# adamgreig/basebandboard

Hardware: AMD Instinct MI355X
Metric: awgn_clt_gsamples_per_s (higher is better)
Workload: dtype u32 bit-sliced GF(2) / int8 out

## Files before the change

basebandboard_amd/_lib.py:

```python
import ctypes as C
import pathlib

import torch

_HERE = pathlib.Path(__file__).resolve().parent
LIB_PATH = _HERE / "libbbb_hip.so"

SHARD_TRIALS, SHARD_SEEDS, SHARD_BITS, SHARD_GROUPS = 0, 1, 2, 3
BBB_OK, BBB_EINVAL, BBB_ENOMEM, BBB_EHIP, BBB_EIO, BBB_ENODEV, BBB_EUNSUP = 0, -1, -2, -3, -4, -5, -6

SYMBOLS = [
    "bbb_abi_version", "bbb_strerror", "bbb_last_error_detail", "bbb_device_count", "bbb_free",
    "bbb_lutopt_load_matrix_file", "bbb_lutopt_create", "bbb_lutopt_destroy", "bbb_lutopt_set_stream",
    "bbb_lutopt_is_specialised", "bbb_lutopt_set_staged", "bbb_lutopt_set_custom_fill", "bbb_lutopt_set_custom_ber", "bbb_lutopt_attach_custom_library", "bbb_lutopt_profile", "bbb_lutopt_profile_read", "bbb_lutopt_profile_read_mover", "bbb_lutopt_state_at", "bbb_lutopt_fill_words", "bbb_awgn_fill_i8", "bbb_awgn_fill_i16", "bbb_awgn_prefetch", "bbb_awgn_stream_open", "bbb_awgn_stream_next", "bbb_awgn_stream_read", "bbb_awgn_stream_seek", "bbb_awgn_stream_tell", "bbb_awgn_stream_close", "bbb_awgn_hist",
    "bbb_clt_tree_i16", "bbb_prbs_fill", "bbb_prbs_fill_hint", "bbb_prbs_check", "bbb_prbs_check_dev", "bbb_prbs_state_at",
    "bbb_prbs_detector_run", "bbb_prbs_detector_stream", "bbb_ber_trials", "bbb_ber_trials_dev", "bbb_ber_run_open", "bbb_ber_run_next", "bbb_ber_run_next_dev", "bbb_ber_run_tell", "bbb_ber_run_close", "bbb_ber_sweep_multi", "bbb_sweep_shard", "bbb_multi_last_info", "bbb_multi_release", "bbb_shaper_fill_i16", "bbb_tx_fill_i16", "bbb_tx_stream_open", "bbb_tx_stream_next", "bbb_tx_stream_read", "bbb_tx_stream_seek", "bbb_tx_stream_tell", "bbb_tx_stream_close", "bbb_rx_slice", "bbb_rx_phase_search", "bbb_eye_accumulate_i16", "bbb_tx_eye_open", "bbb_tx_eye_run", "bbb_tx_eye_close", "bbb_tx_ber_sweep_open", "bbb_tx_ber_sweep_run", "bbb_tx_ber_sweep_close", "bbb_acf_accumulate_i16", "bbb_tx_acf_open", "bbb_tx_acf_run", "bbb_tx_acf_close", "bbb_nco_rom", "bbb_nco_open", "bbb_nco_set_cfg", "bbb_nco_set_stream", "bbb_nco_run", "bbb_nco_get_state", "bbb_nco_set_state", "bbb_nco_close", "bbb_sinc_coefficients", "bbb_sinc_interpolate", "bbb_sinc_eye_open", "bbb_sinc_eye_run", "bbb_sinc_eye_close", "bbb_fir_moving_average", "bbb_fir_filter", "bbb_fir_slice", "bbb_link_sweep_open", "bbb_link_sweep_run", "bbb_link_sweep_close", "bbb_gf2_berlekamp_massey", "bbb_gf2_recur",
    "bbb_gf2_dot", "bbb_gf2_poly_is_primitive", "bbb_gf2_poly_modexp", "bbb_lutopt_charpoly", "bbb_lutopt_is_full_period",
    "bbb_lutopt_save_matrix_file", "bbb_lutopt_search_candidate", "bbb_lutopt_search",
    "bbb_errstat_open", "bbb_errstat_accumulate", "bbb_errstat_skip", "bbb_errstat_read", "bbb_errstat_reset",
    "bbb_errstat_set_stream", "bbb_errstat_geometry", "bbb_errstat_close",
    "bbb_xcorr_accumulate_i16", "bbb_tx_xcorr_open", "bbb_tx_xcorr_run", "bbb_tx_xcorr_close",
    "bbb_ddc_run", "bbb_ddc_polar_host",
    "bbb_dfe_run", "bbb_dfe_geometry", "bbb_dfe_model_host",
]


class BbbError(RuntimeError):
    def __init__(self, code, what, detail):
        super().__init__(f"{what}: {detail}" if detail else what)
        self.code = code


class TrialCfg(C.Structure):
    _fields_ = [("prbs_k", C.c_int32), ("amp", C.c_int32), ("noise_var", C.c_int32), ("reserved", C.c_int32),
                ("prbs_state", C.c_uint64), ("warmup", C.c_uint64), ("first_bit", C.c_uint64),
                ("nbits", C.c_uint64)]

# ... 98 lines not shown
            f"{LIB_PATH} is missing: build it with `python -c 'import __graft_entry__ as g; g.build()'` "
            "(hipcc --offload-arch=gfx950).  basebandboard_amd has no CPU fallback.")
    l = C.CDLL(str(LIB_PATH))
    vp, u64, i32 = C.c_void_p, C.c_uint64, C.c_int
    u64p = C.POINTER(C.c_uint64)
    l.bbb_abi_version.restype = i32
    l.bbb_strerror.restype = C.c_char_p
    l.bbb_strerror.argtypes = [i32]
    l.bbb_last_error_detail.restype = C.c_char_p
    l.bbb_device_count.argtypes = [C.POINTER(i32)]
    l.bbb_free.argtypes = [vp]
    l.bbb_free.restype = None
    l.bbb_lutopt_load_matrix_file.argtypes = [C.c_char_p, C.POINTER(i32), C.POINTER(C.POINTER(C.c_uint16)),
                                              C.POINTER(C.POINTER(C.c_uint32))]
    l.bbb_lutopt_create.argtypes = [C.POINTER(vp), i32, C.POINTER(C.c_uint16), C.POINTER(C.c_uint32), u64p, i32]
    l.bbb_lutopt_destroy.argtypes = [vp]
    l.bbb_lutopt_set_stream.argtypes = [vp, vp]
    l.bbb_lutopt_is_specialised.argtypes = [vp]
    l.bbb_lutopt_set_staged.argtypes = [vp, i32]
    l.bbb_lutopt_state_at.argtypes = [vp, u64, u64p]
    l.bbb_lutopt_profile.argtypes = [vp, i32]
    l.bbb_lutopt_profile_read.argtypes = [vp, C.POINTER(C.c_double), C.POINTER(C.c_double), u64p, i32]
    l.bbb_lutopt_profile_read_mover.argtypes = [vp, C.POINTER(C.c_double), u64p, i32]
    l.bbb_lutopt_fill_words.argtypes = [vp, vp, u64, u64, i32]
    l.bbb_awgn_fill_i8.argtypes = [vp, vp, u64, u64]
    l.bbb_awgn_fill_i16.argtypes = [vp, vp, u64, u64]
    l.bbb_awgn_prefetch.argtypes = [vp, u64, u64]
    l.bbb_awgn_stream_open.argtypes = [vp, u64, u64, i32, C.POINTER(vp)]
    l.bbb_awgn_stream_next.argtypes = [vp, vp]
    l.bbb_awgn_stream_read.argtypes = [vp, vp, u64]
    l.bbb_awgn_stream_seek.argtypes = [vp, u64]
    l.bbb_awgn_stream_tell.argtypes = [vp, u64p]
    l.bbb_awgn_stream_close.argtypes = [vp]
    l.bbb_awgn_hist.argtypes = [vp, vp, u64, u64]
    l.bbb_clt_tree_i16.argtypes = [i32, vp, u64, vp, i32, vp]
    l.bbb_prbs_fill.argtypes = [i32, u64, u64, u64, vp, i32, vp]
    l.bbb_prbs_fill_hint.argtypes = [i32, u64, u64, u64, vp, C.c_uint, i32, vp]
    l.bbb_prbs_check.argtypes = [i32, u64, u64, u64, vp, u64p, i32, vp]
    l.bbb_prbs_check_dev.argtypes = [i32, u64, u64, u64, vp, vp, i32, vp]
    l.bbb_prbs_state_at.argtypes = [i32, u64, u64, u64p]
    l.bbb_prbs_detector_run.argtypes = [i32, vp, u64, u64, vp, vp, i32, vp]
    l.bbb_rx_phase_search.argtypes = [vp, u64, u64, u64, i32, i32, C.POINTER(DetectorStats), i32, vp]
    l.bbb_prbs_detector_stream.argtypes = [i32, vp, u64, vp, vp, C.POINTER(DetectorStats), u64, u64, i32, vp]
    l.bbb_ber_trials.argtypes = [vp, C.POINTER(TrialCfg), i32, C.POINTER(Ber)]
    l.bbb_ber_trials_dev.argtypes = [vp, C.POINTER(TrialCfg), i32, vp]
    l.bbb_multi_last_info.argtypes = [C.POINTER(MultiInfo)]
# ... 140 lines not shown
```

basebandboard_amd/csrc/awgn_kernels.hip:

```cpp
#include "bbb_common.hpp"
#include "bitslice_util.hpp"
#include "awgn_launch.hpp"
#include "stage_common.hpp"

#include <cstdlib>
#include <mutex>
#include <type_traits>
#include "gen/lutopt256_gen.inc"

namespace bbb {


template <int W32, typename TabPtr>
__device__ __forceinline__ void nibble_matvec_part(TabPtr tab, int nlo, int nhi, const uint32_t (&x)[W32],
                                                   uint32_t (&y)[W32]) {
    constexpr int C = (W32 % 4 == 0) ? 4 : (W32 % 2 == 0 ? 2 : 1);
    constexpr int NC = W32 / C;
    typedef uint32_t chunk_t __attribute__((ext_vector_type(C)));
#pragma unroll
    for (int w = 0; w < W32; w++) {
        uint32_t xw = x[w];
        asm volatile("" : "+v"(xw));
#pragma unroll
        for (int q = 0; q < 8; q += 2) {
// ... 587 lines not shown
    __builtin_amdgcn_s_setprio(3);
    uint32_t a[256], b[256], pa[256], pb[256], cnt[8];
    if constexpr (SMALL) {
#ifdef BBB_SMALL_THROTTLE
        asm volatile("" ::: BBB_SMALL_THROTTLE);
#endif
        const uint32_t voff = (uint32_t)LG * 4u;
#define BBB_PLANE(p) (*reinterpret_cast<const uint32_t *>(reinterpret_cast<const char *>(planes + (size_t)(p) * nlanes) + (unsigned long long)voff))
#define BBB_PARK(p) { const uint32_t v_ = BBB_PLANE(p); BBB_ACC_WRITE(pa[p], v_); }
        LUTOPT256_FOR_PARKED_HI(BBB_PARK)
#undef BBB_PARK
#pragma unroll
        for (int p = 0; p < 256; p++)
            if (!lutopt256_hi_is_parked(p)) a[p] = BBB_PLANE(p);
#undef BBB_PLANE
    } else {
#pragma unroll
        for (int p = 0; p < 256; p++) b[p] = planes[(size_t)p * nlanes + LG];
        lutopt256_advance(b, a);
#define BBB_PARK(p) BBB_ACC_WRITE(pa[p], a[p]);
        LUTOPT256_FOR_PARKED_HI(BBB_PARK)
#undef BBB_PARK
    }
    u32x4 *out = stage_row(stage, wave, L, lane);
#pragma unroll 1
    for (unsigned t = 0; t < L; t += 2) {
        lutopt256_step_parked_hi(a, pa, b, pb, cnt);
        {
        __builtin_nontemporal_store((u32x4){cnt[0], cnt[1], cnt[2], cnt[3]}, out);
        __builtin_nontemporal_store((u32x4){cnt[4], cnt[5], cnt[6], cnt[7]}, out + kStageHalfVecs);
        }
        lutopt256_step_parked_hi(b, pb, a, pa, cnt);
        {
        __builtin_nontemporal_store((u32x4){cnt[0], cnt[1], cnt[2], cnt[3]}, out + kStageStepVecs);
        __builtin_nontemporal_store((u32x4){cnt[4], cnt[5], cnt[6], cnt[7]}, out + kStageStepVecs + kStageHalfVecs);
        }
        out += 2 * kStageStepVecs;
    }
}

int awgn256_planes_launch(const uint32_t *d_planes, void *stage, unsigned L, unsigned nlanes, hipStream_t st, bool small_footprint) {
    if (L & 1) return fail(BBB_EINVAL, "segment length must be even");
    if (small_footprint)
        hipLaunchKernelGGL(awgn256_planes_kernel<true>, dim3(nlanes / 64), dim3(64), 0, st, d_planes, (u32x4 *)stage, L, nlanes);
    else
        hipLaunchKernelGGL(awgn256_planes_kernel<false>, dim3(nlanes / 64), dim3(64), 0, st, d_planes, (u32x4 *)stage, L, nlanes);
    BBB_HIP(hipGetLastError());
    return BBB_OK;
}

constexpr unsigned kUnplaneRaw = kStageUnitBytes, kUnplaneLds = 3 * kStageUnitBytes, kUnplaneLdsTx = kUnplaneLds + 32 * 1024 + 2 * 2048;

template <bool TXM, bool NOWRAP = false>
__global__ void __launch_bounds__(256, 7)
unplane_kernel(const u32x4 *__restrict stage, char *__restrict dst, unsigned long long win_lo, unsigned long long nbytes_, unsigned L,
               unsigned long long G, StageGeom ge, TxFuse tx) {
    extern __shared__ __attribute__((aligned(16))) uint32_t lds[];
    typedef __attribute__((address_space(3))) void *lds_void_ptr;
    const unsigned tid = threadIdx.x, lane = tid & 63;
    const unsigned wv = (unsigned)__builtin_amdgcn_readfirstlane((int)(tid >> 6));
    if (blockIdx.x * ge.per_block >= ge.nunits) return;
    char *const dstw = dst - win_lo;
    const unsigned long long nbytes = win_lo + nbytes_;
    const unsigned l8 = tid & 7, qs = tid >> 3;
    const unsigned wr0 = l8 * 32 + ((((qs >> 2) ^ (2 * ((l8 >> 1) & 3))) << 2) | (qs & 3));
    const unsigned lq = (tid >> 3) & 7, c2 = tid & 7;
    const unsigned rd0 = (wv * 8 + lq) * 32 + ((c2 ^ (2 * ((lq >> 1) & 3))) << 2);
    uint32_t *const tile = lds + 2 * (kUnplaneRaw / 4);
    uint32_t *const T10 = lds + kUnplaneLds / 4;
    uint32_t *const winb = lds + kUnplaneLds / 4 + 8192;
    if (TXM) {
        uint16_t *const TT = reinterpret_cast<uint16_t *>(tile);
        for (int e = (int)tid; e < 256 * 8; e += 256) {
            const int q = e >> 3, j = e & 7, ph = (int)((tx.c0 + (unsigned)j) & 7u);
// ... 15 lines not shown
        }
        __syncthreads();
    }
    auto dma_unit = [&](const StagePos &p, unsigned buf) {
        stage_dma_unit(stage, ge, p, L, lds + buf * (kUnplaneRaw / 4), wv, lane);
        if (TXM) {
            const unsigned step0 = p.rg * kStageUnitSteps;
            const unsigned long long wabs = (unsigned long long)ge.w_lo + p.w;
            const long long so = (long long)((wabs * 2048 + p.q8 * 8) * (unsigned long long)L + step0) - (long long)win_lo;
#pragma unroll
            for (unsigned i = 0; i < 2; i++) {
                const unsigned e = (wv * 2 + i) * 64 + lane, row = e >> 1;
                const long long pu = so + (long long)((unsigned long long)((row >> 3) * 64 + (row & 7)) * L);
                uint32_t word = 0;
                if (pu > -128 && pu < (long long)nbytes_) word = (((uint32_t)(pu >> 3) + tx.rel_base) >> 5) + (e & 1);
                word = word < tx.last_word ? word : tx.last_word;
                __builtin_amdgcn_global_load_lds((const void *)(tx.bits + word), (lds_void_ptr)(uintptr_t)(winb + buf * 512 + (wv * 2 + i) * 64), 4, 0, 0);
            }
        }
    };
    auto wait_vm = [](unsigned n) {
        switch (n) {
#define BBB_W(N) case N: asm volatile("s_waitcnt vmcnt(" #N ")" ::: "memory"); break;
            BBB_W(8) BBB_W(10) BBB_W(16) BBB_W(26)
#undef BBB_W
        default: asm volatile("s_waitcnt vmcnt(0)" ::: "memory"); break;
        }
    };
    constexpr unsigned NDMA = TXM ? 10 : 8, NST = TXM ? 16 : 8;
    StagePos cur;
    const unsigned n_it = stage_block_units(ge, blockIdx.x, &cur);
    StagePos nxt = cur;
    stage_advance(nxt, ge);
    unsigned buf = 0;
    bool fast1 = false;
    dma_unit(cur, 0);
    for (unsigned it = 0; it < n_it; it++, buf ^= 1) {
        const unsigned q8 = cur.q8, step0 = cur.rg * 128;
        const unsigned long long w = (unsigned long long)ge.w_lo + cur.w;
        const bool more1 = it + 1 < n_it;
        if (more1) dma_unit(nxt, buf ^ 1);
        wait_vm((more1 ? NDMA : 0u) + (fast1 ? NST : 0u));
        __builtin_amdgcn_s_barrier();
        {
            uint32_t Z[4][8];
            stage_unpack<TXM>(lds + buf * (kUnplaneRaw / 4), tid, Z);
#pragma unroll
            for (unsigned s = 0; s < 4; s++) planes8_to_bytes(Z[s]);
#pragma unroll
            for (unsigned i = 0; i < 8; i++) {
                uint32_t z[4] = {Z[0][i], Z[1][i], Z[2][i], Z[3][i]};
                transpose4x4_bytes(z);
#pragma unroll
                for (unsigned q = 0; q < 4; q++) tile[wr0 + (8 * q + i) * 256] = z[q];
            }
        }
        asm volatile("s_waitcnt lgkmcnt(0)" ::: "memory");
        __builtin_amdgcn_s_barrier();
        const unsigned inseg = step0 + c2 * 16;
        const unsigned long long g0 = (w * 32 + wv) * 64 + q8 * 8 + lq;
        unsigned long long off = g0 * (unsigned long long)L + inseg;
        const unsigned long long goff = 256ull * L;
        const bool lane_fast = inseg < L && g0 + 7 * 256 < G && off >= win_lo && off + 7 * goff + 16 <= nbytes;
        const bool wave_fast = __all(lane_fast);
        fast1 = wave_fast;
        if (!TXM && inseg < L) {
            if (wave_fast) {
#pragma unroll
                for (unsigned k = 0; k < 8; k++) {
// ... 540 lines not shown
```

basebandboard_amd/csrc/bbb_api.hip:

```cpp
#include "bbb_common.hpp"
#include "dev_buf.hpp"
#include "capture.hpp"
#include "awgn_launch.hpp"
#include "stage_common.hpp"
#include "gf2.hpp"
#include "rccl_loader.hpp"
#include "sweep_shard.hpp"
#include "sweep_threads.hpp"

#include <algorithm>
#include <cstdlib>
#include <cstring>
#include <map>
#include <memory>
#include <mutex>
#include <thread>
#include <utility>
#include <vector>

namespace bbb {

std::string &last_error() {
    static thread_local std::string s;
    return s;
// ... 56 lines not shown
        if (read_pending) BBB_HIP(hipEventSynchronize(last_read));
        read_pending = false;
        for (size_t i = 0; i < N; i++)
            if (const int rc = buf[i].grow(need[i])) return rc;
        return BBB_OK;
    }
    int wait_read(hipStream_t s) const {
        if (read_pending) BBB_HIP(hipStreamWaitEvent(s, last_read, 0));
        return BBB_OK;
    }
    int mark_read(hipStream_t s) {
        if (const int rc = last_read.record(s)) return rc;
        read_pending = true;
        return BBB_OK;
    }
};
enum { kStates = 0, kPlanes = 1 };

struct StageSlot {
    DevBuf<uint32_t> stage;
    Event arith;
    Event free;
    bool busy = false;
    uint64_t gen = 0;
    DevBuf<uint32_t> bits[2];
    unsigned bits_turn = 0;

    int grow_stage(size_t words) {
        if (stage.cap >= words) return BBB_OK;
        if (busy) BBB_HIP(hipEventSynchronize(free));
        busy = false;
        return stage.grow(words);
    }
    int grow_bits(unsigned b, size_t words) {
        if (bits[b].cap >= words) return BBB_OK;
        if (busy) BBB_HIP(hipEventSynchronize(free));
        return bits[b].grow(words);
    }
    int wait_free(hipStream_t s) const { if (busy) BBB_HIP(hipStreamWaitEvent(s, free, 0)); return BBB_OK; }
    int mover_queued(hipStream_t ms) {
        if (const int rc = free.record(ms)) return rc;
        busy = true;
        gen++;
        return BBB_OK;
    }
};
// ... 387 lines not shown
}

uint64_t ahead_total(const bbb_lutopt *h, uint64_t n, uint64_t cap, uint64_t step, uint64_t first, uint64_t pos_bound) {
    const uint64_t m = (uint64_t)h->staged_level;
    const bool ahead = m >= 2 && (n % 16) == 0 && m * n < cap && step + m * n >= m * n && (!pos_bound || first + m * n < pos_bound);
    return ahead ? m * n : n;
}

int produce_planes(bbb_lutopt *h, uint64_t L, unsigned nlanes, ProfEv *ev, bool planes_seeded_after_mover, int *slot_out,
                   bool small_footprint = false) {
    const int slot = h->stage_slot ^= 1;
    StageSlot &sl = h->slots[slot];
    *slot_out = slot;
    if (h->ahead.valid && h->ahead.slot == slot) h->ahead.valid = false;
    int rc;
    if ((rc = sl.grow_stage(stage_words(nlanes, L)))) return rc;
    const bool seeding_saw_last_mover = planes_seeded_after_mover && h->pf_waited_slot == slot && h->pf_waited_gen == sl.gen;
    if (planes_seeded_after_mover) h->pf_waited_slot = -1;
    if (!seeding_saw_last_mover && (rc = sl.wait_free(h->cs))) return rc;
    if (ev) BBB_HIP(hipEventRecord(ev->e1, h->cs));
    rc = awgn256_planes_launch(h->cur.buf[kPlanes], (void *)sl.stage.p, (unsigned)L, nlanes, h->cs, small_footprint);
    h->last_staged_small = small_footprint;
    if (rc) return rc;
    if ((rc = mark_planes_read(h))) return rc;
    if (ev) BBB_HIP(hipEventRecord(ev->e2, h->cs));
    return sl.arith.record(h->cs);
}

struct StagedRun { uint64_t L = 0, G = 0; unsigned nlanes = 0; int slot = 0; };

template <typename Hook, typename LaunchMover>
int staged_produce(bbb_lutopt *h, uint64_t ntotal, uint64_t seed_step, bool small_form, bool timed, Hook hook, LaunchMover launch_mover,
                   StagedRun *run) {
    StagedRun &r = *run;
    uint64_t &L = r.L, &G = r.G;
    partition(h, ntotal, 16, &L, &G, &r.nlanes);
    if (L > 0xffffff00ull) return fail(BBB_EINVAL, "nsamples too large for one call (segment length must fit 32 bits): split it");
    int rc = begin_op(h, true, h->pf.matches(seed_step, L, G));
    if (rc) return rc;
    h->last_fill_tx = false;
    ProfEv ev;
    const bool prof = timed && h->profiling;
    if (prof && (rc = ev.begin(h->cs))) return rc;
    bool from_pf = false;
    if ((rc = acquire_planes(h, seed_step, L, G, r.nlanes, true, &from_pf))) return rc;
    if ((rc = hook())) return rc;
// ... 436 lines not shown
        h->prof_prev_e2 = std::move(ev.e2);
        h->prof_seed_ms += a; h->prof_main_ms += b; h->prof_calls++;
    }
    if (seed_ms) *seed_ms = h->prof_seed_ms;
    if (kernel_ms) *kernel_ms = h->prof_main_ms;
    if (calls) *calls = h->prof_calls;
    if (reset) { h->prof_seed_ms = h->prof_main_ms = 0; h->prof_calls = 0; }
    return BBB_OK;
}

int bbb_lutopt_profile_read_mover(bbb_lutopt *h, double *mover_ms, uint64_t *calls, int reset) {
    if (!h) return fail(BBB_EINVAL, "null handle");
    std::vector<std::pair<Event, Event>> pending;
    pending.swap(h->prof_mover_pending);
    for (const auto &ev : pending) {
        BBB_HIP(hipEventSynchronize(ev.second));
        float a = 0;
        BBB_HIP(hipEventElapsedTime(&a, ev.first, ev.second));
        h->prof_mover_ms += a; h->prof_mover_calls++;
    }
    if (mover_ms) *mover_ms = h->prof_mover_ms;
    if (calls) *calls = h->prof_mover_calls;
    if (reset) { h->prof_mover_ms = 0; h->prof_mover_calls = 0; }
    return BBB_OK;
}

int bbb_lutopt_state_at(bbb_lutopt *h, uint64_t nsteps, uint64_t *state_words) {
    if (!h || !state_words) return fail(BBB_EINVAL, "null argument");
    h->pw->apply(nsteps, h->init, state_words);
    return BBB_OK;
}

static int seed_announced(bbb_lutopt *h, uint64_t first_step, uint64_t L, uint64_t G, unsigned nlanes, hipStream_t side, int seed_variant) {
    JumpPlan *plan;
    int rc = get_plan(h, L, &plan);
    if (rc) return rc;
    SeededStates &pf = h->pf;
    pf.valid = false;
    if (pf.seeded) BBB_HIP(hipStreamWaitEvent(side, pf.seeded, 0));
    if ((rc = pf.set.wait_read(side))) return rc;
    if ((rc = pf.set.grow({(size_t)G * h->W32, (size_t)2 * h->k * nlanes}))) return rc;
    pf.set.read_pending = false;
    uint32_t s16[256];
    first16_at(h, *plan, first_step, s16);
    if ((rc = awgn_seed_launch(h->k, plan->d_cols, s16, G, pf.set.buf[kStates], G, nlanes, pf.set.buf[kPlanes], side, h->fast512 ? 1 : 0, seed_variant))) return rc;
    if ((rc = pf.seeded.record(side))) return rc;
// ... 865 lines not shown
```

basebandboard_amd/csrc/hist_kernels.hip:

```cpp
#include "bbb_common.hpp"
#include "bitslice_util.hpp"
#include "stage_common.hpp"

#include <algorithm>
#include <mutex>

namespace bbb {

typedef uint32_t hist_u32x4 __attribute__((ext_vector_type(4)));

constexpr unsigned kHistLanes = 64;
constexpr unsigned kHistRaw = kStageUnitBytes;
constexpr unsigned kHistTable = 256 * kHistLanes * 4;
constexpr unsigned kHistPlanesLds = kHistTable + 2 * kHistRaw;
constexpr int kHistSampleThreads = 1024;

__device__ __forceinline__ uint32_t hist_fold(const uint32_t *H, unsigned bin) {
    uint32_t sum = 0;
    for (unsigned l = 0; l < kHistLanes; l++) sum += H[bin * kHistLanes + ((l + bin) & (kHistLanes - 1))];
    return sum;
}

__global__ void __launch_bounds__(256, 7)
hist_planes_kernel(const hist_u32x4 *__restrict stage, unsigned long long nsamples, unsigned L, StageGeom ge, uint32_t *__restrict scratch) {
    extern __shared__ __attribute__((aligned(16))) uint32_t lds[];
    typedef __attribute__((address_space(3))) void *lds_void_ptr;
    const unsigned tid = threadIdx.x, lane = tid & 63;
    const unsigned wv = (unsigned)__builtin_amdgcn_readfirstlane((int)(tid >> 6));
    uint32_t *const H = lds;
    uint32_t *const raw0 = lds + kHistTable / 4;
    {
        hist_u32x4 *h4 = reinterpret_cast<hist_u32x4 *>(H);
        for (unsigned i = tid; i < kHistTable / 16; i += 256) h4[i] = hist_u32x4{0u, 0u, 0u, 0u};
    }
    __syncthreads();
    const unsigned l8 = tid & 7, qs = tid >> 3;
    const uint32_t hbase = (uint32_t)(uintptr_t)(lds_void_ptr)H;
    const uint32_t column = lane * 4u;
    StagePos cur;
    const unsigned n_it = stage_block_units(ge, blockIdx.x, &cur);
    StagePos nxt = cur;
    stage_advance(nxt, ge);
    unsigned buf = 0;
    if (n_it) stage_dma_unit(stage, ge, cur, L, raw0, wv, lane);
    for (unsigned it = 0; it < n_it; it++, buf ^= 1) {
        const bool more = it + 1 < n_it;
        if (more) stage_dma_unit(stage, ge, nxt, L, raw0 + (buf ^ 1) * (kHistRaw / 4), wv, lane);
        if (more) asm volatile("s_waitcnt vmcnt(8)" ::: "memory");
        else asm volatile("s_waitcnt vmcnt(0)" ::: "memory");
        __builtin_amdgcn_s_barrier();
        {
            uint32_t Z[4][8];
            stage_unpack<true>(raw0 + buf * (kHistRaw / 4), tid, Z);
#pragma unroll
            for (unsigned s = 0; s < 4; s++) planes8_to_bytes(Z[s]);
            const unsigned step = cur.rg * 128 + 4 * qs;
            const unsigned long long span = 64ull * L;
            const unsigned long long off0 = (((unsigned long long)ge.w_lo + cur.w) * kStageWaveGens + cur.q8 * 8 + l8) * L + step;
#define BBB_HIST_ADD(WORD, Q) \
    asm volatile("ds_add_u32 %0, %1" ::"v"(hbase + __builtin_amdgcn_perm(column, (WORD), 0x0c0c0004u | ((Q) << 8))), "v"(1u) : "memory")
            if (step + 3 < L && off0 + 3 + 31 * span < nsamples) {
#pragma unroll
                for (unsigned s = 0; s < 4; s++) {
#pragma unroll
                    for (unsigned i = 0; i < 8; i++) {
                        BBB_HIST_ADD(Z[s][i], 0u); BBB_HIST_ADD(Z[s][i], 1u); BBB_HIST_ADD(Z[s][i], 2u); BBB_HIST_ADD(Z[s][i], 3u);
                    }
                }
            } else {
#pragma unroll
                for (unsigned s = 0; s < 4; s++) {
                    const unsigned long long o = off0 + s;
                    unsigned nj = 0;
                    if (step + s < L && o < nsamples) {
                        const unsigned long long m = (nsamples - o - 1) / span + 1;
                        nj = m < 32 ? (unsigned)m : 32u;
// ... 129 lines not shown
```

basebandboard_amd/csrc/stage_common.hpp:

```cpp
#pragma once

#include <algorithm>
#include <cstddef>
#include <cstdint>

namespace bbb {

constexpr unsigned kStageLaneBytes = 16;
constexpr unsigned kStageHalfBytes = 64 * kStageLaneBytes;
constexpr unsigned kStageStepBytes = 2 * kStageHalfBytes;
constexpr unsigned kStageHalfVecs = kStageHalfBytes / 16, kStageStepVecs = kStageStepBytes / 16;
constexpr unsigned kStageWaveGens = 64 * 32;
constexpr unsigned kStageUnitLanes = 8, kStageUnitSteps = 128;
constexpr unsigned kStageUnitBytes = kStageUnitLanes * kStageUnitSteps * 2 * kStageLaneBytes;

inline size_t stage_words(unsigned nlanes, uint64_t L) { return (size_t)(nlanes / 64) * (size_t)L * (kStageStepBytes / 4); }

struct StageGeom {
    unsigned w_lo, ngroups, nunits;
    unsigned per_block;
};

inline unsigned stage_geom(uint64_t win_lo, uint64_t n, unsigned L, unsigned nlanes, uint64_t blocks_wanted, StageGeom *ge) {
    const uint64_t seg = (uint64_t)L * kStageWaveGens;
    const uint64_t w_lo = win_lo / seg;
    const uint64_t w_hi = std::min<uint64_t>((win_lo + n + seg - 1) / seg, nlanes / 64);
    ge->w_lo = (unsigned)w_lo;
    ge->ngroups = (L + kStageUnitSteps - 1) / kStageUnitSteps;
    const uint64_t nunits = w_hi > w_lo ? (w_hi - w_lo) * ge->ngroups * (64 / kStageUnitLanes) : 0;
    if (nunits == 0 || nunits >> 32) return 0;
    ge->nunits = (unsigned)nunits;
    const uint64_t want = std::max<uint64_t>(1, std::min<uint64_t>(blocks_wanted, nunits));
    ge->per_block = (unsigned)((nunits + want - 1) / want);
    return (unsigned)((nunits + ge->per_block - 1) / ge->per_block);
}

#ifdef __HIPCC__

typedef uint32_t stage_u32x4 __attribute__((ext_vector_type(4)));

__device__ __forceinline__ stage_u32x4 *stage_row(stage_u32x4 *stage, unsigned long long wave, unsigned L, unsigned lane) {
    return stage + (wave * L) * kStageStepVecs + lane;
}

struct StagePos { unsigned q8, rg, w; };

__device__ __forceinline__ void stage_advance(StagePos &p, const StageGeom &ge) {
    if (++p.rg == ge.ngroups) {
        p.rg = 0;
        if (++p.q8 == 64 / kStageUnitLanes) { p.q8 = 0; p.w++; }
    }
}

__device__ __forceinline__ unsigned stage_block_units(const StageGeom &ge, unsigned block, StagePos *first) {
    const unsigned u0 = block * ge.per_block;
    first->rg = u0 % ge.ngroups;
    first->q8 = (u0 / ge.ngroups) & 7;
    first->w = (u0 / ge.ngroups) >> 3;
    return u0 >= ge.nunits ? 0u : (ge.nunits - u0 < ge.per_block ? ge.nunits - u0 : ge.per_block);
}

__device__ __forceinline__ const char *stage_unit_src(const void *stage, unsigned long long wabs, unsigned L, unsigned step0, unsigned q8) {
    return reinterpret_cast<const char *>(stage) + ((wabs * L + step0) * kStageStepVecs + q8 * kStageUnitLanes) * 16;
}

__device__ __forceinline__ void stage_dma_unit(const void *stage, const StageGeom &ge, const StagePos &p, unsigned L, uint32_t *raw, unsigned wv,
                                               unsigned lane) {
    typedef __attribute__((address_space(3))) void *lds_void_ptr;
    const unsigned step0 = p.rg * kStageUnitSteps;
    const char *const sb = stage_unit_src(stage, (unsigned long long)ge.w_lo + p.w, L, step0, p.q8);
    uint32_t *const rawb = raw + wv * 8 * 256;
    if (step0 + kStageUnitSteps <= L) {
        const char *const pl = sb + wv * kStageStepBytes + (lane & 7) * 16 + (lane >> 3) * (4 * kStageStepBytes);
#pragma unroll
        for (unsigned k = 0; k < 8; k++)
            __builtin_amdgcn_global_load_lds((const void *)(pl + ((k & 3) * 32 * kStageStepBytes + (k >> 2) * kStageHalfBytes)),
                                             (lds_void_ptr)(uintptr_t)(rawb + k * 256), 16, 0, 0);
    } else {
        const unsigned last = L - 1 - step0;
#pragma unroll
        for (unsigned k = 0; k < 8; k++) {
            unsigned st = 4 * ((k & 3) * 8 + (lane >> 3)) + wv;
            st = st < last ? st : last;
            __builtin_amdgcn_global_load_lds((const void *)(sb + (size_t)st * kStageStepBytes + (k >> 2) * kStageHalfBytes + (lane & 7) * 16),
                                             (lds_void_ptr)(uintptr_t)(rawb + k * 256), 16, 0, 0);
        }
    }
}

template <bool COMPLEMENT7>
__device__ __forceinline__ void stage_unpack(const uint32_t *raw_image, unsigned tid, uint32_t (&Z)[4][8]) {
    const uint32_t *raw = raw_image + ((tid >> 3) * 8 + (tid & 7)) * 4;
#pragma unroll
    for (unsigned s = 0; s < 4; s++) {
        const stage_u32x4 lo = *reinterpret_cast<const stage_u32x4 *>(raw + (2 * s) * 1024);
        const stage_u32x4 hi = *reinterpret_cast<const stage_u32x4 *>(raw + (2 * s + 1) * 1024);
        Z[s][0] = lo[0]; Z[s][1] = lo[1]; Z[s][2] = lo[2]; Z[s][3] = lo[3];
        Z[s][4] = hi[0]; Z[s][5] = hi[1]; Z[s][6] = hi[2]; Z[s][7] = COMPLEMENT7 ? ~hi[3] : hi[3];
    }
}

#endif

}
```

basebandboard_amd/rng.py:

```python
import ctypes as C

import numpy as np
import torch

from . import _lib, recurrences


def _stream_ptr(device):
    return C.c_void_p(torch.cuda.current_stream(device).cuda_stream)


def _int_to_words(v, k):
    n = (k + 63) // 64
    return (C.c_uint64 * n)(*[(v >> (64 * i)) & 0xFFFFFFFFFFFFFFFF for i in range(n)])


class LUTOPT:

    def __init__(self, a, init=1, device=0):
        a = np.asarray(a)
        if a.ndim != 2 or a.shape[0] != a.shape[1]:
            raise ValueError("recurrence matrix must be square")
        self._setup([np.nonzero(row)[0].tolist() for row in a], init, device)

# ... 99 lines not shown
            out = torch.empty(n, dtype=torch.int32, device=dev)
        if out.dtype != torch.int32 or out.numel() < n or not out.is_contiguous() or out.device != dev:
            raise ValueError(f"out must be a contiguous int32 tensor on {dev} with >= nstates * k/32 elements")
        self._bind_stream()
        _lib.check(_lib.lib().bbb_lutopt_fill_words(self._h, C.c_void_p(out.data_ptr()), int(nstates), int(first_step),
                                                    int(bool(msb_first))), "bbb_lutopt_fill_words")
        return out[:n]

    def profile(self, enable=True):
        _lib.check(_lib.lib().bbb_lutopt_profile(self._h, int(enable)), "bbb_lutopt_profile")

    def profile_read(self, reset=True):
        a, b, n = C.c_double(), C.c_double(), C.c_uint64()
        _lib.check(_lib.lib().bbb_lutopt_profile_read(self._h, C.byref(a), C.byref(b), C.byref(n), int(reset)),
                   "bbb_lutopt_profile_read")
        return a.value, b.value, n.value

    def profile_read_mover(self, reset=True):
        a, n = C.c_double(), C.c_uint64()
        _lib.check(_lib.lib().bbb_lutopt_profile_read_mover(self._h, C.byref(a), C.byref(n), int(reset)),
                   "bbb_lutopt_profile_read_mover")
        return a.value, n.value

    def _bind_stream(self):
        _lib.check(_lib.lib().bbb_lutopt_set_stream(self._h, _stream_ptr(self.device)), "bbb_lutopt_set_stream")

    def __del__(self):
        h = getattr(self, "_h", None)
        if h:
            try:
                _lib.lib().bbb_lutopt_destroy(h)
            except Exception:
                pass
            self._h = None


class CLTGRNG:

    def __init__(self, urng):
        n = urng.k
        if n & (n - 1):
            raise ValueError("urng width must be a power of two")
        self.urng = urng
        self.n = n
        self.dtype = torch.int8 if n <= 256 else torch.int16

# ... 88 lines not shown
```

include/bbb.h:

```cpp
#ifndef BBB_H
#define BBB_H

#include <stddef.h>
#include <stdint.h>

#ifdef __cplusplus
extern "C" {
#endif

#define BBB_OK        0
#define BBB_EINVAL   -1
#define BBB_ENOMEM   -2
#define BBB_EHIP     -3
#define BBB_EIO      -4
#define BBB_ENODEV   -5
#define BBB_EUNSUP   -6

#define BBB_ABI_VERSION 1
#define BBB_MAX_K 512

int bbb_abi_version(void);
const char *bbb_strerror(int code);
const char *bbb_last_error_detail(void);
int bbb_device_count(int *count);
void bbb_free(void *p);


typedef struct bbb_lutopt bbb_lutopt;

int bbb_lutopt_load_matrix_file(const char *path, int *k, uint16_t **taps, uint32_t **row_off);

int bbb_lutopt_create(bbb_lutopt **h, int k, const uint16_t *taps, const uint32_t *row_off,
                      const uint64_t *init_words, int device);
int bbb_lutopt_destroy(bbb_lutopt *h);
int bbb_lutopt_set_stream(bbb_lutopt *h, void *hip_stream);
int bbb_lutopt_is_specialised(const bbb_lutopt *h);

int bbb_lutopt_profile(bbb_lutopt *h, int enable);
int bbb_lutopt_profile_read(bbb_lutopt *h, double *seed_ms, double *kernel_ms, uint64_t *calls, int reset);
int bbb_lutopt_profile_read_mover(bbb_lutopt *h, double *mover_ms, uint64_t *calls, int reset);

int bbb_lutopt_state_at(bbb_lutopt *h, uint64_t nsteps, uint64_t *state_words);

int bbb_lutopt_fill_words(bbb_lutopt *h, uint32_t *dst_dev, uint64_t nstates, uint64_t first_step, int msb_first);

int bbb_awgn_fill_i8(bbb_lutopt *h, int8_t *dst_dev, uint64_t nsamples, uint64_t first_step);
int bbb_awgn_prefetch(bbb_lutopt *h, uint64_t nsamples, uint64_t first_step);
int bbb_lutopt_set_staged(bbb_lutopt *h, int enable);
int bbb_awgn_fill_i16(bbb_lutopt *h, int16_t *dst_dev, uint64_t nsamples, uint64_t first_step);

typedef struct bbb_awgn_stream bbb_awgn_stream;
int bbb_awgn_stream_open(bbb_lutopt *h, uint64_t nsamples_per_call, uint64_t first_step, int elem_bytes, bbb_awgn_stream **s);
int bbb_awgn_stream_next(bbb_awgn_stream *s, void *dst_dev);
int bbb_awgn_stream_read(bbb_awgn_stream *s, void *dst_dev, uint64_t nsamples);
int bbb_awgn_stream_seek(bbb_awgn_stream *s, uint64_t first_step);
int bbb_awgn_stream_tell(const bbb_awgn_stream *s, uint64_t *next_step);
int bbb_awgn_stream_close(bbb_awgn_stream *s);

int bbb_awgn_hist(bbb_lutopt *h, uint64_t *hist_dev, uint64_t nsamples, uint64_t first_step);

int bbb_clt_tree_i16(int k, const uint64_t *states_dev, uint64_t nstates, int16_t *out_dev,
                     int device, void *hip_stream);

// ... 303 lines not shown
```

Measured before the change: 955.4.

## Compress staged CLT counts to seven planes with a flagged side-channel fallback

The staging buffer now stores 7 bit-planes per step instead of 8. Plane 7 is reconstructed as the complement of plane 6, which is valid when the count is not in overflow. Each wave records a flag whenever planes 6 and 7 differ, and a single-block fallback kernel then recomputes the exact sign plane for flagged waves into a side buffer. This cuts staging write and read traffic by about an eighth, at the cost of an extra kernel launch, a scalar flag load in every unpack, and a very slow serial fallback if any wave is ever flagged.

After: 989.7 (median of 6 runs). 3.6% higher.

```diff
diff --git a/basebandboard_amd/_lib.py b/basebandboard_amd/_lib.py
--- a/basebandboard_amd/_lib.py
+++ b/basebandboard_amd/_lib.py
@@ -12,7 +12,7 @@
 SYMBOLS = [
     "bbb_abi_version", "bbb_strerror", "bbb_last_error_detail", "bbb_device_count", "bbb_free",
     "bbb_lutopt_load_matrix_file", "bbb_lutopt_create", "bbb_lutopt_destroy", "bbb_lutopt_set_stream",
-    "bbb_lutopt_is_specialised", "bbb_lutopt_set_staged", "bbb_lutopt_set_custom_fill", "bbb_lutopt_set_custom_ber", "bbb_lutopt_attach_custom_library", "bbb_lutopt_profile", "bbb_lutopt_profile_read", "bbb_lutopt_profile_read_mover", "bbb_lutopt_state_at", "bbb_lutopt_fill_words", "bbb_awgn_fill_i8", "bbb_awgn_fill_i16", "bbb_awgn_prefetch", "bbb_awgn_stream_open", "bbb_awgn_stream_next", "bbb_awgn_stream_read", "bbb_awgn_stream_seek", "bbb_awgn_stream_tell", "bbb_awgn_stream_close", "bbb_awgn_hist",
+    "bbb_lutopt_is_specialised", "bbb_lutopt_set_staged", "bbb_lutopt_set_custom_fill", "bbb_lutopt_set_custom_ber", "bbb_lutopt_attach_custom_library", "bbb_lutopt_profile", "bbb_lutopt_profile_read", "bbb_lutopt_profile_read_mover", "bbb_lutopt_staged_flagged", "bbb_lutopt_state_at", "bbb_lutopt_fill_words", "bbb_awgn_fill_i8", "bbb_awgn_fill_i16", "bbb_awgn_prefetch", "bbb_awgn_stream_open", "bbb_awgn_stream_next", "bbb_awgn_stream_read", "bbb_awgn_stream_seek", "bbb_awgn_stream_tell", "bbb_awgn_stream_close", "bbb_awgn_hist",
     "bbb_clt_tree_i16", "bbb_prbs_fill", "bbb_prbs_fill_hint", "bbb_prbs_check", "bbb_prbs_check_dev", "bbb_prbs_state_at",
     "bbb_prbs_detector_run", "bbb_prbs_detector_stream", "bbb_ber_trials", "bbb_ber_trials_dev", "bbb_ber_run_open", "bbb_ber_run_next", "bbb_ber_run_next_dev", "bbb_ber_run_tell", "bbb_ber_run_close", "bbb_ber_sweep_multi", "bbb_sweep_shard", "bbb_multi_last_info", "bbb_multi_release", "bbb_shaper_fill_i16", "bbb_tx_fill_i16", "bbb_tx_stream_open", "bbb_tx_stream_next", "bbb_tx_stream_read", "bbb_tx_stream_seek", "bbb_tx_stream_tell", "bbb_tx_stream_close", "bbb_rx_slice", "bbb_rx_phase_search", "bbb_eye_accumulate_i16", "bbb_tx_eye_open", "bbb_tx_eye_run", "bbb_tx_eye_close", "bbb_tx_ber_sweep_open", "bbb_tx_ber_sweep_run", "bbb_tx_ber_sweep_close", "bbb_acf_accumulate_i16", "bbb_tx_acf_open", "bbb_tx_acf_run", "bbb_tx_acf_close", "bbb_nco_rom", "bbb_nco_open", "bbb_nco_set_cfg", "bbb_nco_set_stream", "bbb_nco_run", "bbb_nco_get_state", "bbb_nco_set_state", "bbb_nco_close", "bbb_sinc_coefficients", "bbb_sinc_interpolate", "bbb_sinc_eye_open", "bbb_sinc_eye_run", "bbb_sinc_eye_close", "bbb_fir_moving_average", "bbb_fir_filter", "bbb_fir_slice", "bbb_link_sweep_open", "bbb_link_sweep_run", "bbb_link_sweep_close", "bbb_gf2_berlekamp_massey", "bbb_gf2_recur",
     "bbb_gf2_dot", "bbb_gf2_poly_is_primitive", "bbb_gf2_poly_modexp", "bbb_lutopt_charpoly", "bbb_lutopt_is_full_period",
@@ -157,6 +157,7 @@
     l.bbb_lutopt_profile.argtypes = [vp, i32]
     l.bbb_lutopt_profile_read.argtypes = [vp, C.POINTER(C.c_double), C.POINTER(C.c_double), u64p, i32]
     l.bbb_lutopt_profile_read_mover.argtypes = [vp, C.POINTER(C.c_double), u64p, i32]
+    l.bbb_lutopt_staged_flagged.argtypes = [vp, u64p]
     l.bbb_lutopt_fill_words.argtypes = [vp, vp, u64, u64, i32]
     l.bbb_awgn_fill_i8.argtypes = [vp, vp, u64, u64]
     l.bbb_awgn_fill_i16.argtypes = [vp, vp, u64, u64]
diff --git a/basebandboard_amd/csrc/awgn_kernels.hip b/basebandboard_amd/csrc/awgn_kernels.hip
--- a/basebandboard_amd/csrc/awgn_kernels.hip
+++ b/basebandboard_amd/csrc/awgn_kernels.hip
@@ -633,34 +633,114 @@
         LUTOPT256_FOR_PARKED_HI(BBB_PARK)
 #undef BBB_PARK
     }
-    u32x4 *out = stage_row(stage, wave, L, lane);
+    char *out = stage_wave_planes(stage, wave, L);
+    const uint32_t o16 = lane * 16, o8 = 3 * kStageRowBytes + lane * 8;
+    uint32_t ovf = 0;
 #pragma unroll 1
     for (unsigned t = 0; t < L; t += 2) {
         lutopt256_step_parked_hi(a, pa, b, pb, cnt);
+        const uint32_t h4 = cnt[4], h5 = cnt[5], h6 = cnt[6];
+        ovf |= cnt[6] ^ cnt[7];
         {
-        __builtin_nontemporal_store((u32x4){cnt[0], cnt[1], cnt[2], cnt[3]}, out);
-        __builtin_nontemporal_store((u32x4){cnt[4], cnt[5], cnt[6], cnt[7]}, out + kStageHalfVecs);
+        __builtin_nontemporal_store((u32x4){cnt[0], cnt[1], cnt[2], cnt[3]}, reinterpret_cast<u32x4 *>(out + o16));
         }
         lutopt256_step_parked_hi(b, pb, a, pa, cnt);
+        ovf |= cnt[6] ^ cnt[7];
         {
-        __builtin_nontemporal_store((u32x4){cnt[0], cnt[1], cnt[2], cnt[3]}, out + kStageStepVecs);
-        __builtin_nontemporal_store((u32x4){cnt[4], cnt[5], cnt[6], cnt[7]}, out + kStageStepVecs + kStageHalfVecs);
-        }
-        out += 2 * kStageStepVecs;
+        __builtin_nontemporal_store((u32x4){cnt[0], cnt[1], cnt[2], cnt[3]}, reinterpret_cast<u32x4 *>(out + o16 + kStageRowBytes));
+        __builtin_nontemporal_store((u32x4){h4, h5, h6, cnt[4]}, reinterpret_cast<u32x4 *>(out + o16 + 2 * kStageRowBytes));
+        __builtin_nontemporal_store((stage_u32x2){cnt[5], cnt[6]}, reinterpret_cast<stage_u32x2 *>(out + o8));
+        }
+        out += kStagePairBytes;
+    }
+    const bool need7 = __any(ovf != 0);
+    if (lane == 0) stage_flags(stage, nlanes / 64, L)[wave] = need7;
+}
+
+__device__ uint16_t g_plane7_taps[sizeof(LUTOPT256_TAPS) / sizeof(LUTOPT256_TAPS[0])];
+__device__ uint16_t g_plane7_ntaps[256];
+
+__global__ void __launch_bounds__(256, 7)
+plane7_kernel(const uint32_t *__restrict planes, void *stage, unsigned L, unsigned nlanes, int state_is_first_sample) {
+    __shared__ uint32_t xs[2][8][256];
+    const unsigned tid = threadIdx.x, nwaves = nlanes / 64;
+    const uint32_t *const flags = stage_flags(stage, nwaves, L);
+    unsigned mine = 0;
+    for (unsigned w = tid; w < nwaves; w += 256) mine |= flags[w];
+    if (!__syncthreads_or((int)mine)) return;
+    uint32_t *const side = stage_side(stage, nwaves, L);
+    for (unsigned wave = 0; wave < nwaves; wave++) {
+        if (!flags[wave]) continue;
+#pragma unroll 1
+        for (unsigned round = 0; round < 8; round++) {
+            const unsigned lane = round * 8 + (tid >> 5), j = tid & 31;
+#pragma unroll 1
+            for (unsigned w = 0; w < 8; w++) {
+                uint32_t x = 0;
+#pragma unroll 1
+                for (unsigned i = 0; i < 32; i++) x |= ((planes[(size_t)(32 * w + i) * nlanes + wave * 64ull + lane] >> j) & 1u) << i;
+                xs[0][w][tid] = x;
+            }
+            unsigned cur = 0;
+#pragma unroll 1
+            for (unsigned c = 0, t = 0; t < L; c++) {
+                if (c || !state_is_first_sample) {
+                    unsigned e = 0;
+#pragma unroll 1
+                    for (unsigned r = 0; r < 256; r += 32) {
+                        uint32_t y = 0;
+#pragma unroll 1
+                        for (unsigned i = 0; i < 32; i++) {
+                            uint32_t acc = 0;
+#pragma unroll 1
+                            for (unsigned n = g_plane7_ntaps[r + i]; n; n--, e++) {
+                                const unsigned tap = g_plane7_taps[e];
+                                acc ^= xs[cur][tap >> 5][tid] >> (tap & 31);
+                            }
+                            y |= (acc & 1u) << i;
+                        }
+                        xs[cur ^ 1][r >> 5][tid] = y;
+                    }
+                    cur ^= 1;
+                }
+                unsigned T = 0;
+#pragma unroll 1
+                for (unsigned w = 0; w < 8; w++)
+                    T += (unsigned)__builtin_popcount(xs[cur][w][tid] ^ (((0x96u >> w) & 1u) ? ~0x96696996u : 0x96696996u));
+                const unsigned long long b = __ballot((((T - 128u) & 255u) >> 7) != 0);
+                if (j == 0) side[stage_side_word(wave, L, t, lane)] = (uint32_t)(b >> (tid & 32));
+                t++;
+            }
+        }
     }
 }
 
 int awgn256_planes_launch(const uint32_t *d_planes, void *stage, unsigned L, unsigned nlanes, hipStream_t st, bool small_footprint) {
     if (L & 1) return fail(BBB_EINVAL, "segment length must be even");
+    {
+        static std::mutex mu;
+        static bool taps_set[64] = {false};
+        int dev = 0;
+        BBB_HIP(hipGetDevice(&dev));
+        std::lock_guard<std::mutex> g(mu);
+        if (dev < 0 || dev >= 64 || !taps_set[dev]) {
+            BBB_HIP(hipMemcpyToSymbol(HIP_SYMBOL(g_plane7_taps), LUTOPT256_TAPS, sizeof(LUTOPT256_TAPS)));
+            BBB_HIP(hipMemcpyToSymbol(HIP_SYMBOL(g_plane7_ntaps), LUTOPT256_NTAPS, sizeof(LUTOPT256_NTAPS)));
+            if (dev >= 0 && dev < 64) taps_set[dev] = true;
+        }
+    }
     if (small_footprint)
         hipLaunchKernelGGL(awgn256_planes_kernel<true>, dim3(nlanes / 64), dim3(64), 0, st, d_planes, (u32x4 *)stage, L, nlanes);
     else
         hipLaunchKernelGGL(awgn256_planes_kernel<false>, dim3(nlanes / 64), dim3(64), 0, st, d_planes, (u32x4 *)stage, L, nlanes);
     BBB_HIP(hipGetLastError());
-    return BBB_OK;
-}
-
-constexpr unsigned kUnplaneRaw = kStageUnitBytes, kUnplaneLds = 3 * kStageUnitBytes, kUnplaneLdsTx = kUnplaneLds + 32 * 1024 + 2 * 2048;
+    hipLaunchKernelGGL(plane7_kernel, dim3(1), dim3(256), 0, st, d_planes, stage, L, nlanes, small_footprint ? 1 : 0);
+    BBB_HIP(hipGetLastError());
+    return BBB_OK;
+}
+
+constexpr unsigned kUnplaneRaw = kStageUnitBytes, kUnplaneTile = 256 * 128, kUnplaneLds = 2 * kUnplaneRaw + kUnplaneTile;
+constexpr unsigned kUnplaneLdsTx = kUnplaneLds + 32 * 1024 + 2 * 2048;
 
 template <bool TXM, bool NOWRAP = false>
 __global__ void __launch_bounds__(256, 7)
@@ -722,12 +802,12 @@
     auto wait_vm = [](unsigned n) {
         switch (n) {
 #define BBB_W(N) case N: asm volatile("s_waitcnt vmcnt(" #N ")" ::: "memory"); break;
-            BBB_W(8) BBB_W(10) BBB_W(16) BBB_W(26)
+            BBB_W(7) BBB_W(8) BBB_W(9) BBB_W(15) BBB_W(16) BBB_W(25)
 #undef BBB_W
         default: asm volatile("s_waitcnt vmcnt(0)" ::: "memory"); break;
         }
     };
-    constexpr unsigned NDMA = TXM ? 10 : 8, NST = TXM ? 16 : 8;
+    constexpr unsigned NDMA = kStageUnitDmas + (TXM ? 2 : 0), NST = TXM ? 16 : 8;
     StagePos cur;
     const unsigned n_it = stage_block_units(ge, blockIdx.x, &cur);
     StagePos nxt = cur;
@@ -744,7 +824,7 @@
         __builtin_amdgcn_s_barrier();
         {
             uint32_t Z[4][8];
-            stage_unpack<TXM>(lds + buf * (kUnplaneRaw / 4), tid, Z);
+            stage_unpack<TXM>(stage, ge, cur, L, lds + buf * (kUnplaneRaw / 4), tid, Z);
 #pragma unroll
             for (unsigned s = 0; s < 4; s++) planes8_to_bytes(Z[s]);
 #pragma unroll
diff --git a/basebandboard_amd/csrc/bbb_api.hip b/basebandboard_amd/csrc/bbb_api.hip
--- a/basebandboard_amd/csrc/bbb_api.hip
+++ b/basebandboard_amd/csrc/bbb_api.hip
@@ -102,6 +102,7 @@
     Event arith;
     Event free;
     bool busy = false;
+    uint64_t L = 0; unsigned nlanes = 0;
     uint64_t gen = 0;
     DevBuf<uint32_t> bits[2];
     unsigned bits_turn = 0;
@@ -535,6 +536,7 @@
     rc = awgn256_planes_launch(h->cur.buf[kPlanes], (void *)sl.stage.p, (unsigned)L, nlanes, h->cs, small_footprint);
     h->last_staged_small = small_footprint;
     if (rc) return rc;
+    sl.L = L; sl.nlanes = nlanes;
     if ((rc = mark_planes_read(h))) return rc;
     if (ev) BBB_HIP(hipEventRecord(ev->e2, h->cs));
     return sl.arith.record(h->cs);
@@ -1017,6 +1019,21 @@
     if (mover_ms) *mover_ms = h->prof_mover_ms;
     if (calls) *calls = h->prof_mover_calls;
     if (reset) { h->prof_mover_ms = 0; h->prof_mover_calls = 0; }
+    return BBB_OK;
+}
+
+int bbb_lutopt_staged_flagged(bbb_lutopt *h, uint64_t *waves) {
+    if (!h || !waves) return fail(BBB_EINVAL, "null argument");
+    *waves = 0;
+    const StageSlot &sl = h->slots[h->stage_slot];
+    if (!sl.L || !sl.stage.p) return BBB_OK;
+    BBB_HIP(hipSetDevice(h->device));
+    BBB_HIP(hipEventSynchronize(sl.arith));
+    const unsigned nwaves = sl.nlanes / 64;
+    std::vector<uint32_t> flags(nwaves);
+    BBB_HIP(hipMemcpy(flags.data(), reinterpret_cast<const char *>(sl.stage.p) + stage_flags_offset(nwaves, sl.L), nwaves * sizeof(uint32_t),
+                      hipMemcpyDeviceToHost));
+    for (uint32_t f : flags) *waves += f != 0;
     return BBB_OK;
 }
 
diff --git a/basebandboard_amd/csrc/hist_kernels.hip b/basebandboard_amd/csrc/hist_kernels.hip
--- a/basebandboard_amd/csrc/hist_kernels.hip
+++ b/basebandboard_amd/csrc/hist_kernels.hip
@@ -46,12 +46,11 @@
     for (unsigned it = 0; it < n_it; it++, buf ^= 1) {
         const bool more = it + 1 < n_it;
         if (more) stage_dma_unit(stage, ge, nxt, L, raw0 + (buf ^ 1) * (kHistRaw / 4), wv, lane);
-        if (more) asm volatile("s_waitcnt vmcnt(8)" ::: "memory");
-        else asm volatile("s_waitcnt vmcnt(0)" ::: "memory");
+        stage_wait_unit(more);
         __builtin_amdgcn_s_barrier();
         {
             uint32_t Z[4][8];
-            stage_unpack<true>(raw0 + buf * (kHistRaw / 4), tid, Z);
+            stage_unpack<true>(stage, ge, cur, L, raw0 + buf * (kHistRaw / 4), tid, Z);
 #pragma unroll
             for (unsigned s = 0; s < 4; s++) planes8_to_bytes(Z[s]);
             const unsigned step = cur.rg * 128 + 4 * qs;
diff --git a/basebandboard_amd/csrc/stage_common.hpp b/basebandboard_amd/csrc/stage_common.hpp
--- a/basebandboard_amd/csrc/stage_common.hpp
+++ b/basebandboard_amd/csrc/stage_common.hpp
@@ -4,21 +4,50 @@
 #include <cstddef>
 #include <cstdint>
 
+#ifdef __HIPCC__
+#define BBB_STAGE_HD __host__ __device__ __forceinline__
+#else
+#define BBB_STAGE_HD inline
+#endif
+
 namespace bbb {
 
-constexpr unsigned kStageLaneBytes = 16;
-constexpr unsigned kStageHalfBytes = 64 * kStageLaneBytes;
-constexpr unsigned kStageStepBytes = 2 * kStageHalfBytes;
-constexpr unsigned kStageHalfVecs = kStageHalfBytes / 16, kStageStepVecs = kStageStepBytes / 16;
+constexpr unsigned kStagePlanes = 7;
+constexpr unsigned kStageRowBytes = 64 * 16;
+constexpr unsigned kStageRow3Bytes = 64 * 8;
+constexpr unsigned kStagePairBytes = 3 * kStageRowBytes + kStageRow3Bytes;
+constexpr unsigned kStageSideStepBytes = 64 * 4;
 constexpr unsigned kStageWaveGens = 64 * 32;
 constexpr unsigned kStageUnitLanes = 8, kStageUnitSteps = 128;
-constexpr unsigned kStageUnitBytes = kStageUnitLanes * kStageUnitSteps * 2 * kStageLaneBytes;
+constexpr unsigned kStageUnitBytes = kStageUnitLanes * kStageUnitSteps * kStagePlanes * 4;
+#define BBB_STAGE_UNIT_DMAS 7
+constexpr unsigned kStageUnitDmas = BBB_STAGE_UNIT_DMAS;
+static_assert(kStageUnitDmas * 4 * 1024 == kStageUnitBytes, "a unit is 4 waves x kStageUnitDmas x 1 KiB");
 
-inline size_t stage_words(unsigned nlanes, uint64_t L) { return (size_t)(nlanes / 64) * (size_t)L * (kStageStepBytes / 4); }
+BBB_STAGE_HD size_t stage_plane_byte(unsigned step, unsigned plane, unsigned lane) {
+    const size_t pair = (size_t)(step >> 1) * kStagePairBytes;
+    const unsigned s = step & 1;
+    if (plane < 4) return pair + s * kStageRowBytes + lane * 16 + plane * 4;
+    if (s == 0) return pair + 2 * kStageRowBytes + lane * 16 + (plane - 4) * 4;
+    if (plane == 4) return pair + 2 * kStageRowBytes + lane * 16 + 12;
+    return pair + 3 * kStageRowBytes + lane * 8 + (plane - 5) * 4;
+}
+
+BBB_STAGE_HD size_t stage_wave_bytes(uint64_t L) { return (size_t)(L / 2) * kStagePairBytes; }
+BBB_STAGE_HD size_t stage_side_offset(unsigned nwaves, uint64_t L) { return (size_t)nwaves * stage_wave_bytes(L); }
+BBB_STAGE_HD size_t stage_flags_offset(unsigned nwaves, uint64_t L) {
+    return stage_side_offset(nwaves, L) + (size_t)nwaves * (size_t)L * kStageSideStepBytes;
+}
+BBB_STAGE_HD size_t stage_side_word(unsigned long long wave, uint64_t L, unsigned step, unsigned lane) {
+    return ((size_t)wave * (size_t)L + step) * 64 + lane;
+}
+
+inline size_t stage_words(unsigned nlanes, uint64_t L) { return (stage_flags_offset(nlanes / 64, L) + (size_t)(nlanes / 64) * 4) / 4; }
 
 struct StageGeom {
     unsigned w_lo, ngroups, nunits;
     unsigned per_block;
+    unsigned nwaves;
 };
 
 inline unsigned stage_geom(uint64_t win_lo, uint64_t n, unsigned L, unsigned nlanes, uint64_t blocks_wanted, StageGeom *ge) {
@@ -27,6 +56,7 @@
     const uint64_t w_hi = std::min<uint64_t>((win_lo + n + seg - 1) / seg, nlanes / 64);
     ge->w_lo = (unsigned)w_lo;
     ge->ngroups = (L + kStageUnitSteps - 1) / kStageUnitSteps;
+    ge->nwaves = nlanes / 64;
     const uint64_t nunits = w_hi > w_lo ? (w_hi - w_lo) * ge->ngroups * (64 / kStageUnitLanes) : 0;
     if (nunits == 0 || nunits >> 32) return 0;
     ge->nunits = (unsigned)nunits;
@@ -35,12 +65,34 @@
     return (unsigned)((nunits + ge->per_block - 1) / ge->per_block);
 }
 
+BBB_STAGE_HD size_t stage_dma_src(unsigned step0, unsigned pairs, unsigned q8, unsigned wv, unsigned k, unsigned lane) {
+    unsigned pair, off;
+    if (k < 6) {
+        const unsigned qs = wv * 8 + (lane >> 3);
+        pair = 2 * qs + (k < 4 ? k >> 1 : k & 1);
+        off = (k < 4 ? (k & 1) : 2u) * kStageRowBytes + (q8 * kStageUnitLanes + (lane & 7)) * 16;
+    } else {
+        const unsigned qs = (wv & 1) * 16 + (lane >> 2);
+        pair = 2 * qs + (wv >> 1);
+        off = 3 * kStageRowBytes + q8 * kStageUnitLanes * 8 + (lane & 3) * 16;
+    }
+    pair = pair < pairs ? pair : pairs - 1;
+    return (size_t)(step0 / 2 + pair) * kStagePairBytes + off;
+}
+
 #ifdef __HIPCC__
 
 typedef uint32_t stage_u32x4 __attribute__((ext_vector_type(4)));
+typedef uint32_t stage_u32x2 __attribute__((ext_vector_type(2)));
 
-__device__ __forceinline__ stage_u32x4 *stage_row(stage_u32x4 *stage, unsigned long long wave, unsigned L, unsigned lane) {
-    return stage + (wave * L) * kStageStepVecs + lane;
+__device__ __forceinline__ char *stage_wave_planes(void *stage, unsigned long long wave, unsigned L) {
+    return reinterpret_cast<char *>(stage) + wave * stage_wave_bytes(L);
+}
+__device__ __forceinline__ uint32_t *stage_side(void *stage, unsigned nwaves, unsigned L) {
+    return reinterpret_cast<uint32_t *>(reinterpret_cast<char *>(stage) + stage_side_offset(nwaves, L));
+}
+__device__ __forceinline__ uint32_t *stage_flags(void *stage, unsigned nwaves, unsigned L) {
+    return reinterpret_cast<uint32_t *>(reinterpret_cast<char *>(stage) + stage_flags_offset(nwaves, L));
 }
 
 struct StagePos { unsigned q8, rg, w; };
@@ -60,43 +112,60 @@
     return u0 >= ge.nunits ? 0u : (ge.nunits - u0 < ge.per_block ? ge.nunits - u0 : ge.per_block);
 }
 
-__device__ __forceinline__ const char *stage_unit_src(const void *stage, unsigned long long wabs, unsigned L, unsigned step0, unsigned q8) {
-    return reinterpret_cast<const char *>(stage) + ((wabs * L + step0) * kStageStepVecs + q8 * kStageUnitLanes) * 16;
-}
-
 __device__ __forceinline__ void stage_dma_unit(const void *stage, const StageGeom &ge, const StagePos &p, unsigned L, uint32_t *raw, unsigned wv,
                                                unsigned lane) {
     typedef __attribute__((address_space(3))) void *lds_void_ptr;
     const unsigned step0 = p.rg * kStageUnitSteps;
-    const char *const sb = stage_unit_src(stage, (unsigned long long)ge.w_lo + p.w, L, step0, p.q8);
-    uint32_t *const rawb = raw + wv * 8 * 256;
-    if (step0 + kStageUnitSteps <= L) {
-        const char *const pl = sb + wv * kStageStepBytes + (lane & 7) * 16 + (lane >> 3) * (4 * kStageStepBytes);
+    const unsigned pairs = (L - step0 < kStageUnitSteps ? L - step0 : kStageUnitSteps) / 2;
+    const char *const wp = reinterpret_cast<const char *>(stage) + ((unsigned long long)ge.w_lo + p.w) * stage_wave_bytes(L);
 #pragma unroll
-        for (unsigned k = 0; k < 8; k++)
-            __builtin_amdgcn_global_load_lds((const void *)(pl + ((k & 3) * 32 * kStageStepBytes + (k >> 2) * kStageHalfBytes)),
-                                             (lds_void_ptr)(uintptr_t)(rawb + k * 256), 16, 0, 0);
-    } else {
-        const unsigned last = L - 1 - step0;
-#pragma unroll
-        for (unsigned k = 0; k < 8; k++) {
-            unsigned st = 4 * ((k & 3) * 8 + (lane >> 3)) + wv;
-            st = st < last ? st : last;
-            __builtin_amdgcn_global_load_lds((const void *)(sb + (size_t)st * kStageStepBytes + (k >> 2) * kStageHalfBytes + (lane & 7) * 16),
-                                             (lds_void_ptr)(uintptr_t)(rawb + k * 256), 16, 0, 0);
-        }
-    }
+    for (unsigned k = 0; k < kStageUnitDmas; k++)
+        __builtin_amdgcn_global_load_lds((const void *)(wp + stage_dma_src(step0, pairs, p.q8, wv, k, lane)),
+                                         (lds_void_ptr)(uintptr_t)(raw + ((k < 6 ? k * 4 : 24) + wv) * 256), 16, 0, 0);
+}
+
+__device__ __forceinline__ void stage_wait_unit(bool more) {
+#define BBB_STAGE_STR2(x) #x
+#define BBB_STAGE_STR(x) BBB_STAGE_STR2(x)
+    if (more) asm volatile("s_waitcnt vmcnt(" BBB_STAGE_STR(BBB_STAGE_UNIT_DMAS) ")" ::: "memory");
+    else asm volatile("s_waitcnt vmcnt(0)" ::: "memory");
+#undef BBB_STAGE_STR
+#undef BBB_STAGE_STR2
 }
 
 template <bool COMPLEMENT7>
-__device__ __forceinline__ void stage_unpack(const uint32_t *raw_image, unsigned tid, uint32_t (&Z)[4][8]) {
-    const uint32_t *raw = raw_image + ((tid >> 3) * 8 + (tid & 7)) * 4;
+__device__ __forceinline__ void stage_unpack(const void *stage, const StageGeom &ge, const StagePos &p, unsigned L, const uint32_t *raw_image,
+                                             unsigned tid, uint32_t (&Z)[4][8]) {
+    const unsigned qs = tid >> 3, l8 = tid & 7;
+    const uint32_t *raw = raw_image + (qs * 8 + l8) * 4;
 #pragma unroll
     for (unsigned s = 0; s < 4; s++) {
-        const stage_u32x4 lo = *reinterpret_cast<const stage_u32x4 *>(raw + (2 * s) * 1024);
-        const stage_u32x4 hi = *reinterpret_cast<const stage_u32x4 *>(raw + (2 * s + 1) * 1024);
+        const stage_u32x4 lo = *reinterpret_cast<const stage_u32x4 *>(raw + s * 1024);
         Z[s][0] = lo[0]; Z[s][1] = lo[1]; Z[s][2] = lo[2]; Z[s][3] = lo[3];
-        Z[s][4] = hi[0]; Z[s][5] = hi[1]; Z[s][6] = hi[2]; Z[s][7] = COMPLEMENT7 ? ~hi[3] : hi[3];
+    }
+#pragma unroll
+    for (unsigned h = 0; h < 2; h++) {
+        const stage_u32x4 mid = *reinterpret_cast<const stage_u32x4 *>(raw + (4 + h) * 1024);
+        const stage_u32x2 top = *reinterpret_cast<const stage_u32x2 *>(raw_image + 6 * 1024 + (h * 256 + qs * 8 + l8) * 2);
+        Z[2 * h][4] = mid[0]; Z[2 * h][5] = mid[1]; Z[2 * h][6] = mid[2];
+        Z[2 * h + 1][4] = mid[3]; Z[2 * h + 1][5] = top[0]; Z[2 * h + 1][6] = top[1];
+    }
+#pragma unroll
+    for (unsigned s = 0; s < 4; s++) Z[s][7] = COMPLEMENT7 ? ~Z[s][6] : Z[s][6];
+    const unsigned wabs = (unsigned)__builtin_amdgcn_readfirstlane((int)(ge.w_lo + p.w));
+    const uint32_t *const flag_at = stage_flags(const_cast<void *>(stage), ge.nwaves, L) + wabs;
+    uint32_t flag;
+    asm volatile("s_load_dword %0, %1, 0x0\n\ts_waitcnt lgkmcnt(0)" : "=s"(flag) : "s"(flag_at) : "memory");
+    if (flag) {
+        const uint32_t *const side = stage_side(const_cast<void *>(stage), ge.nwaves, L);
+        const unsigned step = p.rg * kStageUnitSteps + 4 * qs;
+        uint32_t w7[4];
+#pragma unroll
+        for (unsigned s = 0; s < 4; s++)
+            w7[s] = __builtin_nontemporal_load(side + stage_side_word(wabs, L, step + s < L ? step + s : L - 1, p.q8 * kStageUnitLanes + l8));
+        asm volatile("s_waitcnt vmcnt(0)" : "+v"(w7[0]), "+v"(w7[1]), "+v"(w7[2]), "+v"(w7[3])::"memory");
+#pragma unroll
+        for (unsigned s = 0; s < 4; s++) Z[s][7] = COMPLEMENT7 ? ~w7[s] : w7[s];
     }
 }
 
diff --git a/basebandboard_amd/rng.py b/basebandboard_amd/rng.py
--- a/basebandboard_amd/rng.py
+++ b/basebandboard_amd/rng.py
@@ -145,6 +145,11 @@
                    "bbb_lutopt_profile_read_mover")
         return a.value, n.value
 
+    def staged_flagged(self):
+        n = C.c_uint64()
+        _lib.check(_lib.lib().bbb_lutopt_staged_flagged(self._h, C.byref(n)), "bbb_lutopt_staged_flagged")
+        return n.value
+
     def _bind_stream(self):
         _lib.check(_lib.lib().bbb_lutopt_set_stream(self._h, _stream_ptr(self.device)), "bbb_lutopt_set_stream")
 
diff --git a/include/bbb.h b/include/bbb.h
--- a/include/bbb.h
+++ b/include/bbb.h
@@ -39,6 +39,7 @@
 int bbb_lutopt_profile(bbb_lutopt *h, int enable);
 int bbb_lutopt_profile_read(bbb_lutopt *h, double *seed_ms, double *kernel_ms, uint64_t *calls, int reset);
 int bbb_lutopt_profile_read_mover(bbb_lutopt *h, double *mover_ms, uint64_t *calls, int reset);
+int bbb_lutopt_staged_flagged(bbb_lutopt *h, uint64_t *waves);
 
 int bbb_lutopt_state_at(bbb_lutopt *h, uint64_t nsteps, uint64_t *state_words);
 
```
